# UtkuKaradeniz/scrabble-gan

Hardware: AMD Instinct MI355X
Metric: train-step images/sec @ 32×160 bs128, 1/2/4/8 GPU; % of HBM/MFMA roofline (higher is better)
Workload: dtype f32

## Files before the change

scrabble_gan_amd/csrc/conv_bf16v2.hip:

```cpp
#include "sg_conv2.h"
#include <stdlib.h>
#include <type_traits>

typedef float f32x16 __attribute__((ext_vector_type(16)));
typedef __bf16 bf16x8 __attribute__((ext_vector_type(8)));
typedef short s16x8 __attribute__((ext_vector_type(8)));
__device__ __attribute__((aligned(256))) unsigned int sg2_zero_page[64];

__device__ __forceinline__ int sg2_xcd_remap(int orig, int nwg) {
  const int q = nwg >> 3, r = nwg & 7, xcd = orig & 7;
  const int base = xcd < r ? xcd * (q + 1) : r * (q + 1) + (xcd - r) * q;
  return base + (orig >> 3);
}

__global__ __launch_bounds__(256) void k_cvt_bf16(const float* __restrict__ x, u16* __restrict__ out, long n8, int relu,
                                                  const float* __restrict__ rowscale, long rowlen) {
  for (long e = (long)blockIdx.x * blockDim.x + threadIdx.x; e < n8; e += (long)gridDim.x * blockDim.x) {
    float4 v0 = reinterpret_cast<const float4*>(x)[2 * e], v1 = reinterpret_cast<const float4*>(x)[2 * e + 1];
    if (rowscale) {
      const float s = rowscale[(8 * e) / rowlen];
      v0.x *= s; v0.y *= s; v0.z *= s; v0.w *= s; v1.x *= s; v1.y *= s; v1.z *= s; v1.w *= s;
    }
    if (relu) {
      v0.x = fmaxf(v0.x, 0.f); v0.y = fmaxf(v0.y, 0.f); v0.z = fmaxf(v0.z, 0.f); v0.w = fmaxf(v0.w, 0.f);
// ... 28 lines not shown
    const int cg = cg0 + cl;
    float s[8] = {0.f, 0.f, 0.f, 0.f, 0.f, 0.f, 0.f, 0.f};
    if (cg < c8) {
      for (long m = m0 + rl; m < m1; m += RL) {
        const float4* src = reinterpret_cast<const float4*>(x + m * C + 8 * cg);
        float4 v0 = src[0], v1 = src[1];
        if (out_plain) {
          bf16x8 hp;
          hp[0] = (__bf16)v0.x; hp[1] = (__bf16)v0.y; hp[2] = (__bf16)v0.z; hp[3] = (__bf16)v0.w;
          hp[4] = (__bf16)v1.x; hp[5] = (__bf16)v1.y; hp[6] = (__bf16)v1.z; hp[7] = (__bf16)v1.w;
          *reinterpret_cast<bf16x8*>(out_plain + m * C + 8 * cg) = hp;
        }
        if (rowscale) {
          const float f = rowscale[m / rows_per_sample];
          v0.x *= f; v0.y *= f; v0.z *= f; v0.w *= f; v1.x *= f; v1.y *= f; v1.z *= f; v1.w *= f;
        }
        bf16x8 hh;
        hh[0] = (__bf16)v0.x; hh[1] = (__bf16)v0.y; hh[2] = (__bf16)v0.z; hh[3] = (__bf16)v0.w;
        hh[4] = (__bf16)v1.x; hh[5] = (__bf16)v1.y; hh[6] = (__bf16)v1.z; hh[7] = (__bf16)v1.w;
        *reinterpret_cast<bf16x8*>(out + m * C + 8 * cg) = hh;
        s[0] += v0.x; s[1] += v0.y; s[2] += v0.z; s[3] += v0.w; s[4] += v1.x; s[5] += v1.y; s[6] += v1.z; s[7] += v1.w;
      }
    }
    if (RL > 1) {
#pragma unroll
      for (int j = 0; j < 8; ++j) red[j * 256 + threadIdx.x] = s[j];
      __syncthreads();
      for (int st = RL >> 1; st > 0; st >>= 1) {
        if (rl < st) {
#pragma unroll
          for (int j = 0; j < 8; ++j) red[j * 256 + threadIdx.x] += red[j * 256 + threadIdx.x + st * CL];
        }
        __syncthreads();
      }
#pragma unroll
      for (int j = 0; j < 8; ++j) s[j] = red[j * 256 + threadIdx.x];
      __syncthreads();
    }
    if (rl == 0 && cg < c8) {
#pragma unroll
      for (int j = 0; j < 8; ++j) atomicAdd(dbias + 8 * cg + j, s[j]);
    }
  }
}

extern "C" int sg_cvt_bf16_bias(const float* x, void* out, void* out_plain, long M, int C, const float* rowscale, long rows_per_sample,
                                float* dbias, void* stream) {
  if (!x || !out || !dbias || M < 0 || C <= 0 || (C & 7) || (rowscale && rows_per_sample <= 0)) return SG_ERR_ARG;
  if (M == 0) return SG_OK;
  long r = (M + 1023) / 1024;
  if (sg_deterministic()) r = M;
  const int rpb = (int)(r < 32 ? 32 : r);
  SG_KERNEL(k_cvt_bf16_bias, dim3((unsigned)((M + rpb - 1) / rpb)), dim3(256), 0, (hipStream_t)stream, x, (u16*)out, (u16*)out_plain, M, C,
                     rowscale, rows_per_sample, dbias, rpb);
  return sg_launch_status();
}

constexpr int SG2_BM = 256, SG2_BK = 64;
constexpr int SG2_TILE = SG2_BM * SG2_BK * 2;
constexpr int SG2_LDS = 4 * SG2_TILE;

template <int BN, int ES, bool RELU, int BMT = 256, int NWO = 0>
__global__ __launch_bounds__((NWO ? NWO : (BMT == 256 ? 8 : 4)) * 64, 2) void sg_igemm_bf16v2_kernel(const SgIgemm2Args p) {
  extern __shared__ __attribute__((aligned(1024))) unsigned char smem[];
  constexpr int BM = BMT, BK = 128 / ES;
  constexpr int NW = NWO ? NWO : (BM == 256 ? 8 : 4);
  constexpr int ATILE = BM * 128;
  constexpr int WN = BN / 64, WM = NW / WN;
  constexpr int TM = BM / WM / 32, TN = 2;
  constexpr int BQ = BN / (8 * NW);
  constexpr int AQ = BM / (8 * NW);
  static_assert(BM == 256 || (BM == 128 && (BN == 128 || (BN == 64 && ES == 4))), "tile configurations");
  static_assert(NWO == 0 || (NWO == 8 && BM == 128 && ES == 4), "eight waves: the fp32 128 x 128 tile only");
  constexpr int BTILE = BN * 128;
  const int tid = threadIdx.x;
  const int lane = tid & 63;
  const int wave = __builtin_amdgcn_readfirstlane(tid >> 6);
  const int wm = wave / WN, wn = wave % WN;

  const int M = p.Bn * p.Hg * p.Wg;
  const int HW = p.Hg * p.Wg;
  const int n_tiles = p.N / BN;
  int wg, split, nsplit;
  if ((int)blockIdx.x < p.full_tiles) {
    wg = sg2_xcd_remap(blockIdx.x, p.full_tiles);
    split = 0;
    nsplit = 1;
  } else {
    const int tail_tiles = p.n_tiles_total - p.full_tiles;
    const int u = sg2_xcd_remap(blockIdx.x - p.full_tiles, tail_tiles * p.tail_split);
    nsplit = p.tail_split;
    split = u / tail_tiles;
    wg = p.full_tiles + (u - split * tail_tiles);
  }
  const int m0 = (wg / n_tiles) * BM;
  const int n0 = (wg % n_tiles) * BN;
  const int grp = p.group_rows ? m0 / p.group_rows : 0;
  const int grp_row0 = grp * p.group_rows;
  const int kchunks = p.Ca / BK;
  const int KT_all = p.ntaps * kchunks;
  const int kt_begin = (int)(((long)KT_all * split) / nsplit);
  const int KT = (int)(((long)KT_all * (split + 1)) / nsplit) - kt_begin;

  const int lrow = lane >> 3, lslot = lane & 7;
  const unsigned char* zero = reinterpret_cast<const unsigned char*>(sg2_zero_page) + 16 * lslot;
  unsigned a_off[4], a_msk[4], b_off[4];
#pragma unroll
  for (int i = 0; i < 4; ++i) {
    const int r = (NW * i + wave) * 8 + lrow;
    const int chunk = lslot ^ ((r >> 1) & 7);
    const int m = m0 + r;
    const bool ok = m < M;
    const int mm = ok ? m - grp_row0 : 0;
    const int b = mm / HW;
    const int rem = mm - b * HW;
    const int yg = rem / p.Wg;
    const int xg = rem - yg * p.Wg;
    const int y = yg * p.a_sy, x = xg * p.a_sx;
    a_off[i] = (unsigned)ES * (unsigned)(((b * p.Ha + y) * p.Wa + x) * p.Ca) + 16u * chunk;
    unsigned mk = 0;
    for (int t = 0; t < p.ntaps; ++t) {
      const int iy = y + p.taps[t].dy, ix = x + p.taps[t].dx;
      if (ok && iy >= 0 && iy < p.Ha && ix >= 0 && ix < p.Wa) mk |= 1u << t;
    }
    a_msk[i] = mk;
    b_off[i] = (unsigned)ES * (unsigned)((n0 + (r % BN)) * p.Ca) + 16u * chunk;
  }
  int tab_a = 0, tab_w = 0;
  if (lane < p.ntaps) {
    tab_a = ES * (p.taps[lane].dy * p.Wa + p.taps[lane].dx) * p.Ca;
    tab_w = ES * p.taps[lane].w_off;
  }
  int lt = kt_begin % p.ntaps, lc0 = (kt_begin / p.ntaps) * BK;
  int lidx = 0;
  int cur_a = 0, cur_w = 0;
  unsigned cur_bit = 0;
  bool cur_live = true;
  auto set_cursor = [&]() {
    cur_live = lidx < KT;
    cur_a = __builtin_amdgcn_readlane(tab_a, lt) + ES * lc0;
    cur_w = __builtin_amdgcn_readlane(tab_w, lt) + ES * lc0;
    cur_bit = cur_live ? (1u << lt) : 0u;
  };
  set_cursor();
  auto advance = [&]() {
    ++lidx;
    ++lt;
    const bool wrap = lt >= p.ntaps;
    lt = wrap ? 0 : lt;
    lc0 += wrap ? BK : 0;
    set_cursor();
  };
  const unsigned long long a_base64 = (unsigned long long)reinterpret_cast<uintptr_t>(p.a) + (unsigned long long)grp * (unsigned long long)p.a_group_bytes;
  const unsigned long long z_base64 = (unsigned long long)reinterpret_cast<uintptr_t>(zero);
  const unsigned long long w_base64 = (unsigned long long)reinterpret_cast<uintptr_t>(p.w) + (unsigned long long)grp * (unsigned long long)p.w_group_bytes;
  auto issue_part = [&](int st, int q) {
    const bool ok = (a_msk[q] & cur_bit) != 0;
    const unsigned long long pa = a_base64 + (unsigned long long)(a_off[q] + (unsigned)cur_a);
    const unsigned lo = ok ? (unsigned)pa : (unsigned)z_base64;
    const unsigned hi = ok ? (unsigned)(pa >> 32) : (unsigned)(z_base64 >> 32);
    const unsigned char* src_a = reinterpret_cast<const unsigned char*>((uintptr_t)(((unsigned long long)hi << 32) | lo));
    const unsigned long long pb = cur_live ? w_base64 + (unsigned long long)(b_off[q] + (unsigned)cur_w) : z_base64;
    const unsigned char* src_b = reinterpret_cast<const unsigned char*>((uintptr_t)pb);
    unsigned char* dst_a = smem + st * ATILE + (NW * q + wave) * 1024;
    unsigned char* dst_b = smem + 2 * ATILE + st * BTILE + (NW * q + wave) * 1024;
    if (q < AQ)
      __builtin_amdgcn_global_load_lds((const __attribute__((address_space(1))) void*)src_a, (__attribute__((address_space(3))) void*)dst_a, 16, 0, 0);
    if (q < BQ)
      __builtin_amdgcn_global_load_lds((const __attribute__((address_space(1))) void*)src_b, (__attribute__((address_space(3))) void*)dst_b, 16, 0, 0);
  };

  f32x16 acc[TM][TN];
#pragma unroll
// ... 284 lines not shown
            idx = ((size_t)(b * p.Ho + yg * p.o_sy + p.o_oy) * p.Wo + xg * p.o_sx + p.o_ox) * p.N + n;
          }
          float v = acc[i][j][r] * oscale + bs;
          if (p.mask16) {
            if ((short)p.mask16[idx] <= 0) v = 0.f;
          } else if (p.mask && p.mask[idx] <= 0.f) {
            v = 0.f;
          }
          atomicAdd(p.out + idx, v);
        }
      }
    }
    return;
  }
#pragma unroll
  for (int i = 0; i < TM; ++i) {
    size_t idx[8];
    bool live[8];
    float4 mk32[8], prev[8];
    uint2 mk16[8];
#pragma unroll
    for (int it = 0; it < 8; ++it) {
      const int m = m0 + wm * (TM * 32) + i * 32 + 4 * it + rsub;
      live[it] = m < M;
      const int mm = live[it] ? m : 0;
      if (ident) {
        idx[it] = (size_t)mm * p.N + ncol;
      } else {
        const int b = mm / HW;
        const int rem = mm - b * HW;
        const int yg = rem / p.Wg;
        const int xg = rem - yg * p.Wg;
        idx[it] = ((size_t)(b * p.Ho + yg * p.o_sy + p.o_oy) * p.Wo + xg * p.o_sx + p.o_ox) * p.N + ncol;
      }
      if (p.mask16) mk16[it] = *reinterpret_cast<const uint2*>(p.mask16 + idx[it]);
      else if (p.mask) mk32[it] = *reinterpret_cast<const float4*>(p.mask + idx[it]);
      if (accum) prev[it] = *reinterpret_cast<const float4*>(p.out + idx[it]);
    }
#pragma unroll
    for (int j = 0; j < TN; ++j)
#pragma unroll
      for (int r = 0; r < 16; ++r) stage[((r & 3) + 8 * (r >> 2) + 4 * khalf) * 64 + j * 32 + (lane & 31)] = acc[i][j][r];
#pragma unroll
    for (int it = 0; it < 8; ++it) {
      float4 v = *reinterpret_cast<const float4*>(stage + (4 * it + rsub) * 64 + 4 * c4);
      if (!live[it]) continue;
      v.x = v.x * oscale + bsum.x; v.y = v.y * oscale + bsum.y; v.z = v.z * oscale + bsum.z; v.w = v.w * oscale + bsum.w;
      if (p.mask16) {
        if ((short)(mk16[it].x & 0xffffu) <= 0) v.x = 0.f;
        if ((short)(mk16[it].x >> 16) <= 0) v.y = 0.f;
        if ((short)(mk16[it].y & 0xffffu) <= 0) v.z = 0.f;
        if ((short)(mk16[it].y >> 16) <= 0) v.w = 0.f;
      } else if (p.mask) {
        if (mk32[it].x <= 0.f) v.x = 0.f;
        if (mk32[it].y <= 0.f) v.y = 0.f;
        if (mk32[it].z <= 0.f) v.z = 0.f;
        if (mk32[it].w <= 0.f) v.w = 0.f;
      }
      if (accum) { v.x += prev[it].x; v.y += prev[it].y; v.z += prev[it].z; v.w += prev[it].w; }
      if (relu_out) { v.x = fmaxf(v.x, 0.f); v.y = fmaxf(v.y, 0.f); v.z = fmaxf(v.z, 0.f); v.w = fmaxf(v.w, 0.f); }
      typedef __bf16 bf16x4v __attribute__((ext_vector_type(4)));
      bf16x4v h;
      if (p.out16) { h[0] = (__bf16)v.x; h[1] = (__bf16)v.y; h[2] = (__bf16)v.z; h[3] = (__bf16)v.w; }
      if (p.amax_out) {
        const float4 q = p.out ? v : make_float4((float)h[0], (float)h[1], (float)h[2], (float)h[3]);
        const float a4 = fmaxf(fmaxf(fabsf(q.x), fabsf(q.y)), fmaxf(fabsf(q.z), fabsf(q.w)));
        amx = fmaxf(amx, a4);
        if (p.amax_rowscale) amx_s = fmaxf(amx_s, a4 * fabsf(p.amax_rowscale[(m0 + wm * (TM * 32) + i * 32 + 4 * it + rsub) / HW]));
      }
      if (p.out) *reinterpret_cast<float4*>(p.out + idx[it]) = v;
      if (p.out16) *reinterpret_cast<bf16x4v*>(p.out16 + idx[it]) = h;
    }
  }
  if (p.amax_out) {
    amx = sg_wave_max(amx);
    amx_s = p.amax_rowscale ? sg_wave_max(amx_s) : amx;
    if (lane == 0) {
      sg_atomic_max_nonneg(p.amax_out, amx);
      sg_atomic_max_nonneg(p.amax_out + 1, amx_s);
    }
  }
}

__global__ __launch_bounds__(256) void k_amax_rows(const float* __restrict__ x, long rows, int N, long row0, const float* __restrict__ rowscale,
                                                   long rows_per_sample, unsigned* amax_bits) {
  const int n4 = N >> 2;
  const long total = rows * n4;
  float m0 = 0.f, m1 = 0.f;
  for (long e = (long)blockIdx.x * blockDim.x + threadIdx.x; e < total; e += (long)gridDim.x * blockDim.x) {
    const float4 v = reinterpret_cast<const float4*>(x)[e];
    const float a = fmaxf(fmaxf(fabsf(v.x), fabsf(v.y)), fmaxf(fabsf(v.z), fabsf(v.w)));
    m0 = fmaxf(m0, a);
    m1 = fmaxf(m1, rowscale ? a * fabsf(rowscale[(row0 + e / n4) / rows_per_sample]) : a);
  }
  m0 = sg_wave_max(m0);
  m1 = sg_wave_max(m1);
  if ((threadIdx.x & 63) == 0) {
    sg_atomic_max_nonneg(reinterpret_cast<float*>(amax_bits), m0);
    sg_atomic_max_nonneg(reinterpret_cast<float*>(amax_bits) + 1, m1);
  }
}

static int g2_split_override = -1;
extern "C" void sg_debug_set_splitk_v2(int n) { g2_split_override = n; }

template <int BN, int ES, bool RELU, int BMT = 256, int NWO = 0>
static int sg2_launch_bn_r(SgIgemm2Args a, hipStream_t s, long* twin_rows_done) {
  const long M = (long)a.Bn * a.Hg * a.Wg;
  const int n_tiles = a.N / BN;
  const int tiles = sg_cdiv(M, BMT) * n_tiles;
  if (tiles <= 0) return SG_OK;
  const int KT_all = a.ntaps * (a.Ca / (128 / ES));
  const bool can_split = a.out && !(a.flags & SG_RELU_OUT) && ((a.flags & SG_ACCUM) || (a.flags & SG2_IDENT_OUT));
  constexpr int CUS = BMT == 256 ? 256 : 512;
  int full = tiles, nsplit = 1;
  if (can_split && g2_split_override != 1 && KT_all >= 8) {
    const int rem = tiles % CUS;
    if (g2_split_override > 1) {
      full = 0;
      nsplit = g2_split_override < KT_all ? g2_split_override : 1;
    } else if (rem > 0) {
      const int full_c = tiles < 2 * CUS ? 0 : (tiles - rem) / n_tiles * n_tiles;
      const int tail = tiles - full_c;
      auto cost = [&](int sp) { return (double)((tail * sp + CUS - 1) / CUS) / sp * (1.0 + 0.03 * (sp - 1)); };
      int best = 1;
      double best_cost = cost(1);
      const int sp_max = KT_all / 4 < 16 ? KT_all / 4 : 16;
      for (int sp = 2; sp <= sp_max; ++sp) {
        const double c = cost(sp);
        if (c < 0.97 * best_cost) { best = sp; best_cost = c; }
      }
      if (best > 1) { full = full_c; nsplit = best; }
    }
  }
  const long row0 = nsplit > 1 ? (long)(full / n_tiles) * BMT : M;
  if (nsplit > 1 && !(a.flags & SG_ACCUM)) {
    if (hipMemsetAsync(a.out + (size_t)row0 * a.N, 0, sizeof(float) * (size_t)(M - row0) * a.N, s) != hipSuccess) return SG_ERR_LAUNCH;
  }
  a.full_tiles = full;
  a.tail_split = nsplit;
  a.n_tiles_total = tiles;
  static bool attr_done = false;
  static const int lds_pad = getenv("SG2_LDS_PAD") ? atoi(getenv("SG2_LDS_PAD")) : 0;
  const int LDS_BYTES = 2 * BMT * 128 + 2 * BN * 128 + lds_pad;
  if (!attr_done) {
    if (hipFuncSetAttribute(reinterpret_cast<const void*>(sg_igemm_bf16v2_kernel<BN, ES, RELU, BMT, NWO>), hipFuncAttributeMaxDynamicSharedMemorySize, LDS_BYTES) != hipSuccess) {
      (void)hipGetLastError();
      return SG_ERR_UNSUPPORTED;
    }
    attr_done = true;
  }
  SG_KERNEL((sg_igemm_bf16v2_kernel<BN, ES, RELU, BMT, NWO>), dim3(full + (tiles - full) * nsplit), dim3((NWO ? NWO : (BMT == 256 ? 8 : 4)) * 64), LDS_BYTES, s, a);
  if (twin_rows_done) *twin_rows_done = (a.flags & SG2_IDENT_OUT) ? row0 : (nsplit > 1 ? 0 : M);
  if (a.amax_out && nsplit > 1) {
    const bool ident = (a.flags & SG2_IDENT_OUT) != 0;
    const long r0 = ident ? row0 : 0, nrows = ident ? M - row0 : (long)a.Bn * a.Ho * a.Wo;
    const long per_sample = ident ? (long)a.Hg * a.Wg : (long)a.Ho * a.Wo;
    SG_KERNEL(k_amax_rows, dim3(sg_grid_for(nrows * (a.N / 4), 256)), dim3(256), 0, s, a.out + (size_t)r0 * a.N, nrows, a.N, r0,
                       a.amax_rowscale, per_sample, reinterpret_cast<unsigned*>(a.amax_out));
  }
  return sg_launch_status();
}

template <int BN, int ES, int BMT = 256, int NWO = 0>
static int sg2_launch_bn(const SgIgemm2Args& a, hipStream_t s, long* twin_rows_done) {
  if constexpr (ES == 1) return sg2_launch_bn_r<BN, ES, false, BMT>(a, s, twin_rows_done);
  else return (a.flags & SG_RELU_IN) ? sg2_launch_bn_r<BN, ES, true, BMT, NWO>(a, s, twin_rows_done) : sg2_launch_bn_r<BN, ES, false, BMT, NWO>(a, s, twin_rows_done);
}

static int g2_tile128 = getenv("SG2_TILE128") ? atoi(getenv("SG2_TILE128")) : 0;
extern "C" void sg_debug_set_tile128(int mode) { g2_tile128 = mode; }
static bool sg2_prefer_128(const SgIgemm2Args& a, long m_tiles) {
  return a.ntaps == 1 && a.Ca >= 1024 && m_tiles <= 1024;
}

int sg_launch_igemm_bf16v2(const SgIgemm2Args& a_in, hipStream_t s, long* twin_rows_done, int es) {
  SgIgemm2Args a = a_in;
  if ((a.Ca % (128 / es)) || (a.N % 64) || a.ntaps < 1 || a.ntaps > SG_MAX_TAPS) return SG_ERR_UNSUPPORTED;
  if (es == 1 && ((a.N % 256) || !a.amax_a || !a.amax_w)) return SG_ERR_UNSUPPORTED;
  if (a.group_rows && ((a.group_rows % 128) || a.ntaps != 1 || a.Ha != 1 || a.Wa != 1 || a.Hg != 1 || a.Wg != 1 || a.Ho != 1 || a.Wo != 1 || a.out16 ||
                       a.mask || a.mask16 || a.amax_out || (long)a.Bn % a.group_rows))
    return SG_ERR_ARG;
  const long a_bytes = (long)es * (a.group_rows ? a.group_rows : a.Bn) * a.Ha * a.Wa * a.Ca;
  long w_elems = 0;
  for (int t = 0; t < a.ntaps; ++t) w_elems = a.taps[t].w_off > w_elems ? a.taps[t].w_off : w_elems;
  w_elems += (long)a.N * a.Ca;
  if (a_bytes >= (1L << 32) - 64 || es * w_elems >= (1L << 32) - 64 || (!a.group_rows && (long)a.Bn * a.Ho * a.Wo * a.N >= (1L << 31)) ||
      (long)a.Bn * a.Hg * a.Wg >= (1L << 31) - 256)
    return SG_ERR_UNSUPPORTED;
  if (a.o_sy == 1 && a.o_sx == 1 && a.o_oy == 0 && a.o_ox == 0 && a.Ho == a.Hg && a.Wo == a.Wg) a.flags |= SG2_IDENT_OUT;
  const long m_tiles = sg_cdiv((long)a.Bn * a.Hg * a.Wg, SG2_BM);
  const bool can_split = a.out && !(a.flags & SG_RELU_OUT) && ((a.flags & SG_ACCUM) || (a.flags & SG2_IDENT_OUT)) && a.ntaps * (a.Ca / (128 / es)) >= 8;
  int bn = 0;
  double best = 1e30;
  for (int c = 256; c >= 64; c >>= 1) {
    if (a.N % c) continue;
    const long tiles = m_tiles * (a.N / c);
    const double rounds = can_split && tiles % 256 ? (tiles < 256 ? 1.0 : (double)tiles / 256.0) : (double)((tiles + 255) / 256);
    const double t_tile = es == 4 ? (c == 256 ? 1.0 : c == 128 ? 0.525 : 0.29) : es == 1 ? (c == 256 ? 1.0 : c == 128 ? 0.8 : 0.7)
                                                                                        : (c == 256 ? 1.0 : c == 128 ? 0.75 : 0.625);
    if (rounds * t_tile < 0.97 * best) { best = rounds * t_tile; bn = c; }
  }
  static const int bn_env = getenv("SG2_FORCE_BN") ? atoi(getenv("SG2_FORCE_BN")) : 0;
  if (bn_env > 0 && a.N % bn_env == 0) bn = bn_env;
  if (es == 1) {
    if (bn == 256) return sg2_launch_bn<256, 1>(a, s, twin_rows_done);
    if (bn == 128) return sg2_launch_bn<128, 1>(a, s, twin_rows_done);
    return sg2_launch_bn<64, 1>(a, s, twin_rows_done);
  }
  if (es == 4) {
    static const int w8 = getenv("SG2_W8") ? atoi(getenv("SG2_W8")) : 1;
    const long g_tiles = (long)sg_cdiv((long)a.Bn * a.Hg * a.Wg, 128) * (a.N / 128);
    if (a.group_rows && a.N % 128 == 0 && (w8 == 2 || (w8 == 1 && g_tiles < 8 * 512))) return sg2_launch_bn<128, 4, 128, 8>(a, s, twin_rows_done);
    if (a.group_rows && a.N % 128) return a.N % 64 == 0 ? sg2_launch_bn<64, 4, 128>(a, s, twin_rows_done) : SG_ERR_UNSUPPORTED;
    if (a.group_rows) return sg2_launch_bn<128, 4, 128>(a, s, twin_rows_done);
    if (bn == 256) return sg2_launch_bn<256, 4>(a, s, twin_rows_done);
    if (bn == 128) return sg2_launch_bn<128, 4>(a, s, twin_rows_done);
    return sg2_launch_bn<64, 4>(a, s, twin_rows_done);
  }
  if (a.N % 128 == 0 && bn >= 128 && (g2_tile128 == 2 || (g2_tile128 == 1 && sg2_prefer_128(a, m_tiles)))) return sg2_launch_bn<128, 2, 128>(a, s, twin_rows_done);
  if (bn == 256) return sg2_launch_bn<256, 2>(a, s, twin_rows_done);
  if (bn == 128) return sg2_launch_bn<128, 2>(a, s, twin_rows_done);
  return sg2_launch_bn<64, 2>(a, s, twin_rows_done);
}

static int finish_twin(const SgIgemm2Args& a, long rows_done, hipStream_t s) {
  if (!a.out16) return SG_OK;
  const long M = (long)a.Bn * a.Ho * a.Wo;
  if (rows_done >= M) return SG_OK;
  const long n = (M - rows_done) * a.N;
  SG_KERNEL(k_cvt_bf16, dim3(sg_grid_for(n / 8, 256)), dim3(256), 0, s, a.out + (size_t)rows_done * a.N,
                     a.out16 + (size_t)rows_done * a.N, n / 8, 0, (const float*)nullptr, 8L);
  return sg_launch_status();
}

extern "C" int sg_conv2d_fwd_bf16v2(const void* x16, const void* wp_fwd, const float* bias, const float* bias2, float* y, void* y16,
                                    int B, int H, int W, int Cin, int Cout, int kh, int kw, int pad_same, int flags, float* amax_y,
                                    void* stream) {
  if (!x16 || !wp_fwd || (!y && !y16) || (!y && (flags & SG_ACCUM)) || kh * kw > SG_MAX_TAPS) return SG_ERR_ARG;
  const int ph = pad_same ? kh / 2 : 0, pw = pad_same ? kw / 2 : 0;
  const int Ho = pad_same ? H : H - kh + 1, Wo = pad_same ? W : W - kw + 1;
  SgIgemm2Args a{};
  a.a = (const u16*)x16; a.w = (const u16*)wp_fwd; a.out = y; a.out16 = (u16*)y16; a.bias = bias; a.bias2 = bias2; a.mask = nullptr;
  a.amax_out = amax_y;
  a.Bn = B; a.Ha = H; a.Wa = W; a.Ca = Cin; a.Hg = Ho; a.Wg = Wo; a.a_sy = 1; a.a_sx = 1;
  a.Ho = Ho; a.Wo = Wo; a.N = Cout; a.o_sy = 1; a.o_sx = 1; a.o_oy = 0; a.o_ox = 0;
  a.ntaps = kh * kw; a.flags = flags;
  for (int ky = 0; ky < kh; ++ky)
    for (int kx = 0; kx < kw; ++kx) a.taps[ky * kw + kx] = SgTap{ky - ph, kx - pw, (ky * kw + kx) * Cin * Cout};
  long done = 0;
  const int rc = sg_launch_igemm_bf16v2(a, (hipStream_t)stream, &done, 2);
  return rc != SG_OK ? rc : finish_twin(a, done, (hipStream_t)stream);
}

extern "C" int sg_conv2d_bwd_data_bf16v2(const void* dy16, const void* wp_bwd, const float* mask, const void* mask16, float* dx, void* dx16,
                                         int B, int H, int W, int Cin, int Cout, int kh, int kw, int pad_same, int flags, float* amax_dx,
                                         const float* amax_rowscale, void* stream) {
  if (!dy16 || !wp_bwd || !dx || kh * kw > SG_MAX_TAPS) return SG_ERR_ARG;
  const int ph = pad_same ? kh / 2 : 0, pw = pad_same ? kw / 2 : 0;
  const int Ho = pad_same ? H : H - kh + 1, Wo = pad_same ? W : W - kw + 1;
  SgIgemm2Args a{};
  a.a = (const u16*)dy16; a.w = (const u16*)wp_bwd; a.out = dx; a.out16 = (u16*)dx16; a.mask = mask; a.mask16 = (const u16*)mask16;
  a.amax_out = amax_dx; a.amax_rowscale = amax_rowscale;
  a.Bn = B; a.Ha = Ho; a.Wa = Wo; a.Ca = Cout; a.Hg = H; a.Wg = W; a.a_sy = 1; a.a_sx = 1;
  a.Ho = H; a.Wo = W; a.N = Cin; a.o_sy = 1; a.o_sx = 1;
  a.ntaps = kh * kw; a.flags = flags;
  for (int ky = 0; ky < kh; ++ky)
    for (int kx = 0; kx < kw; ++kx) a.taps[ky * kw + kx] = SgTap{ph - ky, pw - kx, (ky * kw + kx) * Cin * Cout};
  long done = 0;
  const int rc = sg_launch_igemm_bf16v2(a, (hipStream_t)stream, &done, 2);
  return rc != SG_OK ? rc : finish_twin(a, done, (hipStream_t)stream);
}

extern "C" int sg_conv2d_fwd_v2(const float* x, const float* wt_fwd, const float* bias, const float* bias2, float* y, int B, int H,
                                int W, int Cin, int Cout, int kh, int kw, int pad_same, int flags, void* stream) {
  if (!x || !wt_fwd || !y || kh * kw > SG_MAX_TAPS) return SG_ERR_ARG;
  const int ph = pad_same ? kh / 2 : 0, pw = pad_same ? kw / 2 : 0;
  const int Ho = pad_same ? H : H - kh + 1, Wo = pad_same ? W : W - kw + 1;
  SgIgemm2Args a{};
  a.a = (const u16*)x; a.w = (const u16*)wt_fwd; a.out = y; a.bias = bias; a.bias2 = bias2;
  a.Bn = B; a.Ha = H; a.Wa = W; a.Ca = Cin; a.Hg = Ho; a.Wg = Wo; a.a_sy = 1; a.a_sx = 1;
  a.Ho = Ho; a.Wo = Wo; a.N = Cout; a.o_sy = 1; a.o_sx = 1; a.o_oy = 0; a.o_ox = 0;
  a.ntaps = kh * kw; a.flags = flags;
  for (int ky = 0; ky < kh; ++ky)
    for (int kx = 0; kx < kw; ++kx) a.taps[ky * kw + kx] = SgTap{ky - ph, kx - pw, (ky * kw + kx) * Cin * Cout};
  return sg_launch_igemm_bf16v2(a, (hipStream_t)stream, nullptr, 4);
}

extern "C" int sg_conv2d_bwd_data_v2(const float* dy, const float* w, const float* mask, float* dx, int B, int H, int W, int Cin,
                                     int Cout, int kh, int kw, int pad_same, int flags, void* stream) {
  if (!dy || !w || !dx || kh * kw > SG_MAX_TAPS) return SG_ERR_ARG;
  const int ph = pad_same ? kh / 2 : 0, pw = pad_same ? kw / 2 : 0;
  const int Ho = pad_same ? H : H - kh + 1, Wo = pad_same ? W : W - kw + 1;
  SgIgemm2Args a{};
// ... 524 lines not shown
```

scrabble_gan_amd/csrc/sg_conv2.h:

```cpp
#pragma once
#include "sg_conv.h"

typedef unsigned short u16;

#define SG2_IDENT_OUT 32

struct SgIgemm2Args {
  const u16* a;
  const u16* w;
  float* out;
  u16* out16;
  const float* bias;
  const float* bias2;
  const float* mask;
  const u16* mask16;
  const float* amax_a;
  const float* amax_w;
  float* amax_out;
  const float* amax_rowscale;
  int Bn, Ha, Wa, Ca;
  int Hg, Wg, a_sy, a_sx;
  int Ho, Wo, N, o_sy, o_sx, o_oy, o_ox;
  int ntaps, flags;
  int full_tiles, tail_split, n_tiles_total;
  int group_rows;
  long a_group_bytes, w_group_bytes;
  SgTap taps[SG_MAX_TAPS];
};

int sg_launch_igemm_bf16v2(const SgIgemm2Args& a_in, hipStream_t s, long* twin_rows_done, int es);
```

scrabble_gan_amd/ops.py:

```python
from __future__ import annotations

import os as _os
from typing import Optional, Tuple

import torch

from ._lib import call, lib

RELU_IN, ACCUM, RELU_OUT, TANH_OUT = 1, 2, 4, 8
MMA_BF16 = 256
BN_EPS = 1e-3


class KernelTimer:

    def __init__(self, only=None):
        self.records = {}
        self.shapes = {}
        self.nbytes = {}
        self.only = only
        self.roof = {}

    def wants(self, family):
        return self.only is None or any(family.startswith(p) for p in self.only)
# ... 551 lines not shown
    _chk(t, rowscale, db)
    out = torch.empty(t.shape, device=t.device, dtype=torch.bfloat16)
    plain = torch.empty(t.shape, device=t.device, dtype=torch.bfloat16) if want_plain else None
    C = t.shape[-1]
    M = t.numel() // C
    with _hbm("cvt_bf16", t, out, plain):
        call("sg_cvt_bf16_bias", _p(t), out.data_ptr(), None if plain is None else plain.data_ptr(), M, C, _p(rowscale),
             (M // rowscale.numel()) if rowscale is not None else 1, _p(db), _stream())
    return (out, plain) if want_plain else out


def grad_operand(dy: torch.Tensor, sample_scale, want_colsum: bool):
    key = (dy.untyped_storage().data_ptr(), 0 if sample_scale is None else sample_scale.data_ptr(), dy.storage_offset(), dy.numel())
    e = _TWINS.get(key)
    plain = _twin_get(dy)
    if e is None or (want_colsum and e[3] is None):
        whole = dy.storage_offset() == 0 and dy.numel() * 4 == dy.untyped_storage().nbytes()
        colsum = torch.zeros(dy.shape[-1], device=dy.device, dtype=torch.float32)
        if sample_scale is None:
            t16 = cvt_bf16_bias(dy, None, colsum)
            if plain is None:
                _twin_put(dy, t16)
        elif plain is None and whole:
            t16, p16 = cvt_bf16_bias(dy, sample_scale, colsum, want_plain=True)
            _twin_put(dy, p16)
        else:
            t16 = cvt_bf16_bias(dy, sample_scale, colsum)
        e = (dy, sample_scale, t16, colsum)
        _TWINS[key] = e
    return e[2], e[3]


def bf16_of(t: torch.Tensor) -> torch.Tensor:
    t16 = _twin_get(t)
    if t16 is None:
        t16 = cvt_bf16(t)
        _twin_put(t, t16)
    return t16


USE_F32_V2 = _os.environ.get("SG_F32_V2", "1") == "1"


F32_V2_MIN_TILES = 512


def _f32v2_ok(K: int, N: int, kh: int, kw: int, same: bool, pixels: int) -> bool:
    if not (USE_F32_V2 and CONV_DTYPE == "f32" and K % 32 == 0 and N % 64 == 0 and (same or (kh == 1 and kw == 1))):
        return False
    tiles = -(-pixels // 256) * -(-N // 256)
    return tiles >= F32_V2_MIN_TILES and (F32_V2_MIN_TILES == 0 or kh * kw * K >= 1024)


USE_WINOGRAD = _os.environ.get("SG_WINOGRAD", "1") == "1"
WINO_TILE = int(_os.environ.get("SG_WINO_TILE", "4"))
WINO_MIN_C = {2: int(_os.environ.get("SG_WINO_MIN_C", "128")), 4: int(_os.environ.get("SG_WINO4_MIN_C", "64"))}
WINO_MIN_KN = {2: int(_os.environ.get("SG_WINO_MIN_KN", "32768")), 4: int(_os.environ.get("SG_WINO4_MIN_KN", "16384"))}
WINO4_WGRAD_MIN_TILES = 128
_WINO_WS = {}
WINO_KEEP_V = _os.environ.get("SG_WINO_KEEP_V", "1") == "1"
_WINO_V = {"on": False, "map": {}}


def _wino_v_get(x: torch.Tensor, relu_in: bool, tile: int):
    e = _WINO_V["map"].get(x.untyped_storage().data_ptr())
    if e is None or e[1] != relu_in or e[2] != tile or e[0].shape[1:] != x.shape[1:]:
        return None
    per = x.shape[1] * x.shape[2] * x.shape[3]
    off = x.storage_offset() - e[0].storage_offset()
    if off < 0 or off % per or off // per + x.shape[0] > e[0].shape[0]:
        return None
    t0 = (off // per) * (x.shape[1] // tile) * (x.shape[2] // tile)
    if e[5] != _stream():
        e[3].record_stream(torch.cuda.current_stream())
    return e[3].data_ptr() + 4 * t0 * x.shape[3], e[4]


def _wino_tile(H: int, W: int) -> int:
    return 4 if (WINO_TILE == 4 and H % 4 == 0 and W % 4 == 0) else 2


WINO_ROW_GAIN = float(_os.environ.get("SG_WINO_ROW_GAIN", "0.75"))
WINO_N_MULT = int(_os.environ.get("SG_WINO_N_MULT", "64"))


def _wino_rows_ok(B, H: int, W: int, tile: int) -> bool:
    if B is None or WINO_ROW_GAIN <= 0 or DETERMINISTIC:
        return True
    T = B * (H // tile) * (W // tile)
    return (tile + 2) ** 2 * (-(-T // 128) * 128) <= WINO_ROW_GAIN * 9 * (-(-(B * H * W) // 128) * 128)


def _wino_ok(K: int, N: int, kh: int, kw: int, same: bool, H: int, W: int, B=None) -> bool:
    if not (USE_WINOGRAD and CONV_DTYPE == "f32" and kh == 3 and kw == 3 and same and H % 2 == 0 and W % 2 == 0 and K % 32 == 0 and N % WINO_N_MULT == 0):
        return False
    t = _wino_tile(H, W)
    return min(K, N) >= WINO_MIN_C[t] and K * N >= WINO_MIN_KN[t] and _wino_rows_ok(B, H, W, t)


def _wino_workspace(nbytes: int, like: torch.Tensor) -> torch.Tensor:
    key = _stream()
    buf = _WINO_WS.get(key)
    if buf is None or buf.numel() < nbytes:
        _WINO_WS.pop(key, None)
        buf = None
        buf = torch.empty(nbytes, device=like.device, dtype=torch.uint8)
        _WINO_WS[key] = buf
    return buf


def _wino_conv(a, w, out, bias, bias2, mask, K: int, N: int, relu_in: bool, flags: int, tag, ups: bool = False) -> None:
    B, H, W, _ = a.shape
    if ups:
        H, W = 2 * H, 2 * W
        flags |= UPS2_IN
    tile = _wino_tile(H, W)
    P = (tile + 2) ** 2
    fwd = tag[0] == "wino_fwd"
    u = packed_filter(w, ("wino_fwd%d" if fwd else "wino_bwd%d") % tile)
    T = B * (H // tile) * (W // tile)
    Tp = -(-T // 128) * 128
    nbytes = 4 * P * Tp * (K + N)
    s = _stream()
    keep = (fwd and _WINO_V["on"] and a.storage_offset() == 0 and _wino_wgrad_ok(K, N, 3, 3, True, H, W)
            and (tile == 2 or T >= WINO4_WGRAD_MIN_TILES))
    if keep:
        Vt = torch.empty(P * Tp * K, device=a.device, dtype=torch.float32)
        if len(_WINO_V["map"]) > 256:
            _WINO_V["map"].clear()
        _WINO_V["map"][a.untyped_storage().data_ptr()] = (a, bool(relu_in), tile, Vt, Tp, s)
        V = Vt.data_ptr()
        Mt = _wino_workspace(4 * P * Tp * N, a).data_ptr()
        if PROFILER is None:
            call("sg_wino_input", _p(a), V, B, H, W, K, int(relu_in), tile, s)
            call("sg_wino_gemm", V, _p(u), Mt, B, H, W, K, N, tile, s)
            call("sg_wino_output", Mt, _p(out), _p(bias), _p(bias2), None, B, H, W, N, flags, tile, s)
            return
    else:
        ws = _wino_workspace(nbytes, a)
        V = ws.data_ptr()
        Mt = V + 4 * P * Tp * K
    if PROFILER is None:
        if fwd:
            call("sg_conv2d_fwd_wino", _p(a), _p(u), _p(bias), _p(bias2), _p(out), B, H, W, K, N, flags | (1 if relu_in else 0), tile, V, nbytes, s)
        else:
            call("sg_conv2d_bwd_data_wino", _p(a), _p(u), _p(mask), _p(out), B, H, W, N, K, flags, tile, V, nbytes, s)
        return
    with _hbm("wino_transform", a, flops=0.0) as _:
        if PROFILER is not None and PROFILER.wants("wino_transform"):
            PROFILER.nbytes["wino_transform"] = PROFILER.nbytes.get("wino_transform", 0.0) + 4.0 * P * T * K
        if ups:
            call("sg_wino_input_ups", _p(a), V, B, H, W, K, tile, s)
        else:
            call("sg_wino_input", _p(a), V, B, H, W, K, int(relu_in), tile, s)
    with _timed("igemm_wino", 2.0 * P * Tp * K * N, False, tag):
        if PROFILER is not None and PROFILER.wants("igemm_wino"):
            PROFILER.nbytes["igemm_wino"] = PROFILER.nbytes.get("igemm_wino", 0.0) + 4.0 * P * (Tp * K + N * K + Tp * N)
        call("sg_wino_gemm", V, _p(u), Mt, B, H, W, K, N, tile, s)
    with _hbm("wino_transform", out, mask, flops=0.0):
        if PROFILER is not None and PROFILER.wants("wino_transform"):
            PROFILER.nbytes["wino_transform"] = PROFILER.nbytes.get("wino_transform", 0.0) + 4.0 * P * T * N
        call("sg_wino_output", Mt, _p(out), _p(bias), _p(bias2), _p(mask), B, H, W, N, flags & ~UPS2_IN, tile, s)


def _wino_wgrad_ok(Cin: int, Cout: int, kh: int, kw: int, same: bool, H: int, W: int) -> bool:
    if not (USE_WINOGRAD and CONV_DTYPE == "f32" and not DETERMINISTIC and kh == 3 and kw == 3 and same and H % 2 == 0 and W % 2 == 0
# ... 790 lines not shown
```

Baseline: 937.8.

## Add persistent fp32 kernel for Winograd batched GEMMs with cross-tile prefetch

Adds a persistent kernel for fp32 grouped single-tap GEMMs, the Winograd batched products. It is enabled by default and launches at most two workgroups per CU. Each workgroup loops over 128x128 output tiles and prefetches the next tile's first K chunks while storing the current tile's output. This hides per-tile prologue and epilogue latency and launch overhead, and any split-K tail is offset via block0 to the existing kernel. The cost is added complexity and possible load imbalance with the static tile stride.

```diff
diff --git a/scrabble_gan_amd/csrc/conv_bf16v2.hip b/scrabble_gan_amd/csrc/conv_bf16v2.hip
--- a/scrabble_gan_amd/csrc/conv_bf16v2.hip
+++ b/scrabble_gan_amd/csrc/conv_bf16v2.hip
@@ -134,13 +134,15 @@
   const int HW = p.Hg * p.Wg;
   const int n_tiles = p.N / BN;
   int wg, split, nsplit;
-  if ((int)blockIdx.x < p.full_tiles) {
-    wg = sg2_xcd_remap(blockIdx.x, p.full_tiles);
+  int bid = (int)blockIdx.x;
+  if constexpr (ES == 4 && BMT == 128) bid += p.block0;
+  if (bid < p.full_tiles) {
+    wg = sg2_xcd_remap(bid, p.full_tiles);
     split = 0;
     nsplit = 1;
   } else {
     const int tail_tiles = p.n_tiles_total - p.full_tiles;
-    const int u = sg2_xcd_remap(blockIdx.x - p.full_tiles, tail_tiles * p.tail_split);
+    const int u = sg2_xcd_remap(bid - p.full_tiles, tail_tiles * p.tail_split);
     nsplit = p.tail_split;
     split = u / tail_tiles;
     wg = p.full_tiles + (u - split * tail_tiles);
@@ -591,6 +593,192 @@
   }
 }
 
+template <int NW>
+__global__ __launch_bounds__(NW * 64, 2) void sg_wino_persist_kernel(const SgIgemm2Args p) {
+  extern __shared__ __attribute__((aligned(1024))) unsigned char smem[];
+  typedef unsigned long long u64;
+  constexpr int BM = 128, BN = 128, BK = 32;
+  constexpr int ATILE = BM * 128, BTILE = BN * 128;
+  constexpr int WN = BN / 64, WM = NW / WN;
+  constexpr int TM = BM / WM / 32, TN = 2;
+  constexpr int NQ = BM / (8 * NW);
+  constexpr int RP = 128 / NW;
+  static_assert(NW == 4 || NW == 8, "four or eight waves");
+  const int tid = threadIdx.x;
+  const int lane = tid & 63;
+  const int wave = __builtin_amdgcn_readfirstlane(tid >> 6);
+  const int wm = wave / WN, wn = wave % WN;
+  const int n_tiles = p.N / BN;
+  const int KT = p.Ca / BK;
+  const int KT2 = (KT + 1) & ~1;
+  const int grid = (int)gridDim.x;
+
+  auto coords = [&](int vb, int& m0, int& n0, int& grp) {
+    const int wg = sg2_xcd_remap(vb, p.full_tiles);
+    const int mt = wg / n_tiles;
+    m0 = mt * BM;
+    n0 = (wg - mt * n_tiles) * BN;
+    grp = m0 / p.group_rows;
+  };
+  auto bases = [&](int vb, u64& a64, u64& b64, bool& live) {
+    live = vb < p.full_tiles;
+    int m0, n0, grp;
+    coords(live ? vb : 0, m0, n0, grp);
+    a64 = (u64)reinterpret_cast<uintptr_t>(p.a) + (u64)grp * (u64)p.a_group_bytes + 4ull * (u64)(m0 - grp * p.group_rows) * (u64)p.Ca;
+    b64 = (u64)reinterpret_cast<uintptr_t>(p.w) + (u64)grp * (u64)p.w_group_bytes + 4ull * (u64)n0 * (u64)p.Ca;
+  };
+
+  const int lrow = lane >> 3, lslot = lane & 7;
+  const int r0 = wave * 8 + lrow;
+  const unsigned l_off = 4u * (unsigned)(r0 * p.Ca) + 16u * (unsigned)(lslot ^ ((r0 >> 1) & 7));
+  const unsigned qstride = 4u * (unsigned)(NW * 8 * p.Ca);
+  const unsigned z_off = 16u * (unsigned)lslot;
+  const u64 z_base64 = (u64)reinterpret_cast<uintptr_t>(sg2_zero_page);
+
+  int lvb = (int)blockIdx.x, lk = 0;
+  u64 a_cur, b_cur, nx_a, nx_b;
+  bool t_live, nx_live;
+  bases(lvb, a_cur, b_cur, t_live);
+  bases(lvb + grid, nx_a, nx_b, nx_live);
+  bool cur_live = t_live;
+  auto advance = [&]() {
+    ++lk;
+    const bool wrap = lk >= KT2;
+    lk = wrap ? 0 : lk;
+    lvb = wrap ? lvb + grid : lvb;
+    a_cur = wrap ? nx_a : a_cur;
+    b_cur = wrap ? nx_b : b_cur;
+    t_live = wrap ? nx_live : t_live;
+    cur_live = t_live && lk < KT;
+  };
+  auto issue_part = [&](int st, int q) {
+    const u64 kb = (u64)(unsigned)(lk * 128);
+    const u64 sa = cur_live ? a_cur + kb : z_base64;
+    const u64 sb = cur_live ? b_cur + kb : z_base64;
+    const unsigned off = cur_live ? l_off + (unsigned)q * qstride : z_off;
+    const unsigned char* src_a = reinterpret_cast<const unsigned char*>((uintptr_t)(sa + off));
+    const unsigned char* src_b = reinterpret_cast<const unsigned char*>((uintptr_t)(sb + off));
+    unsigned char* dst_a = smem + st * ATILE + (NW * q + wave) * 1024;
+    unsigned char* dst_b = smem + 2 * ATILE + st * BTILE + (NW * q + wave) * 1024;
+    __builtin_amdgcn_global_load_lds((const __attribute__((address_space(1))) void*)src_a, (__attribute__((address_space(3))) void*)dst_a, 16, 0, 0);
+    __builtin_amdgcn_global_load_lds((const __attribute__((address_space(1))) void*)src_b, (__attribute__((address_space(3))) void*)dst_b, 16, 0, 0);
+  };
+
+  f32x16 acc[TM][TN];
+  const int frow = lane & 31, khalf = lane >> 5, swz = (frow >> 1) & 7;
+  const unsigned lds0 = (unsigned)(uintptr_t)(__attribute__((address_space(3))) unsigned char*)smem;
+  typedef float v2f __attribute__((ext_vector_type(2)));
+  unsigned a4[8], b4[8];
+#pragma unroll
+  for (int s = 0; s < 8; ++s) {
+    const unsigned ko = 16u * (unsigned)(s ^ swz) + 8u * (unsigned)khalf;
+    a4[s] = lds0 + (unsigned)((wm * (TM * 32) + frow) * 128) + ko;
+    b4[s] = lds0 + (unsigned)(2 * ATILE + (wn * 64 + frow) * 128) + ko;
+  }
+  v2f af4[2][4], bf4[2][2];
+  auto mma4 = [&](int slot) {
+#pragma unroll
+    for (int e = 0; e < 2; ++e)
+#pragma unroll
+      for (int i = 0; i < TM; ++i)
+#pragma unroll
+        for (int j = 0; j < TN; ++j) acc[i][j] = __builtin_amdgcn_mfma_f32_32x32x2f32(af4[slot][i][e], bf4[slot][j][e], acc[i][j], 0, 0, 0);
+  };
+  auto mma4_dma = [&](int slot, int st) {
+#pragma unroll
+    for (int e = 0; e < 2; ++e)
+#pragma unroll
+      for (int i = 0; i < TM; ++i) {
+#pragma unroll
+        for (int j = 0; j < TN; ++j) acc[i][j] = __builtin_amdgcn_mfma_f32_32x32x2f32(af4[slot][i][e], bf4[slot][j][e], acc[i][j], 0, 0, 0);
+        if (e == 0) {
+          __builtin_amdgcn_sched_barrier(0);
+#pragma unroll
+          for (int q = i * NQ / TM; q < (i + 1) * NQ / TM; ++q) issue_part(st, q);
+          __builtin_amdgcn_sched_barrier(0);
+        }
+      }
+    advance();
+  };
+#define SG4_K_TILE_LAST(st, sn)                                                              \
+  do {                                                                                       \
+    SG4_STEP(st, 1, 1, 0);                                                                   \
+    SG4_STEP(st, 2, 0, 1);                                                                   \
+    SG4_STEP(st, 3, 1, 0);                                                                   \
+    SG4_STEP(st, 4, 0, 1);                                                                   \
+    SG4_STEP(st, 5, 1, 0);                                                                   \
+    SG4_STEP(st, 6, 0, 1);                                                                   \
+    SG4_STEP(st, 7, 1, 0);                                                                   \
+    asm volatile("s_waitcnt vmcnt(0) lgkmcnt(0)" ::: "memory");                              \
+    __builtin_amdgcn_s_barrier();                                                            \
+    SG4_READ_FRAGS(sn, 0, 0);                                                                \
+    __builtin_amdgcn_sched_barrier(0);                                                       \
+    mma4(1);                                                                                 \
+    __builtin_amdgcn_sched_barrier(0);                                                       \
+    asm volatile("s_waitcnt lgkmcnt(0)" ::: "memory");                                       \
+    __builtin_amdgcn_sched_barrier(0);                                                       \
+  } while (0)
+
+  const int sbyte = wave * (RP * 256);
+  float* stage = reinterpret_cast<float*>(smem + (sbyte < ATILE ? ATILE + sbyte : 2 * ATILE + BTILE + (sbyte - ATILE)));
+  const int c4 = lane & 15, rsub = lane >> 4;
+
+  {
+#pragma unroll
+    for (int q = 0; q < NQ; ++q) issue_part(0, q);
+    advance();
+    asm volatile("s_waitcnt vmcnt(0)" ::: "memory");
+    __builtin_amdgcn_s_barrier();
+#pragma unroll
+    for (int q = 0; q < NQ; ++q) issue_part(1, q);
+    advance();
+    SG4_READ_FRAGS(0, 0, 0);
+  }
+  for (int cvb = (int)blockIdx.x;; cvb += grid) {
+    bases(lvb + grid, nx_a, nx_b, nx_live);
+#pragma unroll
+    for (int i = 0; i < TM; ++i)
+#pragma unroll
+      for (int j = 0; j < TN; ++j)
+#pragma unroll
+        for (int r = 0; r < 16; ++r) acc[i][j][r] = 0.f;
+    for (int kt = 2; kt < KT2; kt += 2) {
+      SG4_K_TILE(0, 1);
+      SG4_K_TILE(1, 0);
+    }
+    SG4_K_TILE(0, 1);
+    SG4_K_TILE_LAST(1, 0);
+
+    int m0, n0, grp;
+    coords(cvb, m0, n0, grp);
+    float* out_t = p.out + ((size_t)m0 * p.N + n0);
+#pragma unroll
+    for (int ps = 0; ps < 2; ++ps) {
+      constexpr int NR = NW == 4 ? 16 : 8;
+      const int i = NW == 4 ? ps : 0, rb = NW == 4 ? 0 : 8 * ps;
+#pragma unroll
+      for (int j = 0; j < TN; ++j)
+#pragma unroll
+        for (int rr = 0; rr < NR; ++rr) stage[((rr & 3) + 8 * (rr >> 2) + 4 * khalf) * 64 + j * 32 + (lane & 31)] = acc[i][j][rb + rr];
+#pragma unroll
+      for (int it = 0; it < RP / 4; ++it) {
+        float4 v = *reinterpret_cast<const float4*>(stage + (4 * it + rsub) * 64 + 4 * c4);
+        v.x += 0.f; v.y += 0.f; v.z += 0.f; v.w += 0.f;
+        const int row = wm * (TM * 32) + ps * RP + 4 * it + rsub;
+        *reinterpret_cast<float4*>(out_t + ((size_t)row * p.N + wn * 64 + 4 * c4)) = v;
+      }
+    }
+    if (cvb + grid >= p.full_tiles) break;
+    asm volatile("s_waitcnt lgkmcnt(0)" ::: "memory");
+    __builtin_amdgcn_s_barrier();
+    __builtin_amdgcn_sched_barrier(0);
+#pragma unroll
+    for (int q = 0; q < NQ; ++q) issue_part(1, q);
+    advance();
+    __builtin_amdgcn_sched_barrier(0);
+  }
+}
+
 __global__ __launch_bounds__(256) void k_amax_rows(const float* __restrict__ x, long rows, int N, long row0, const float* __restrict__ rowscale,
                                                    long rows_per_sample, unsigned* amax_bits) {
   const int n4 = N >> 2;
@@ -612,6 +800,20 @@
 
 static int g2_split_override = -1;
 extern "C" void sg_debug_set_splitk_v2(int n) { g2_split_override = n; }
+
+static int g2_wino_persist = getenv("SG_WINO_PERSIST") ? atoi(getenv("SG_WINO_PERSIST")) : 1;
+static int g2_wino_persist_wgs = getenv("SG_WINO_PERSIST_WGS") ? atoi(getenv("SG_WINO_PERSIST_WGS")) : 0;
+extern "C" void sg_debug_set_wino_persist(int mode, int wgs) {
+  g2_wino_persist = mode;
+  g2_wino_persist_wgs = wgs;
+}
+static bool sg2_wino_persist_wanted(const SgIgemm2Args& a, long M) {
+  if (g2_wino_persist <= 0) return false;
+  if (!a.group_rows || a.ntaps != 1 || a.flags != SG2_IDENT_OUT || !a.out || a.out16 || a.bias || a.bias2 || a.mask || a.mask16 || a.amax_out ||
+      (M % 128) || (a.N % 128) || (a.Ca % 32))
+    return false;
+  return true;
+}
 
 template <int BN, int ES, bool RELU, int BMT = 256, int NWO = 0>
 static int sg2_launch_bn_r(SgIgemm2Args a, hipStream_t s, long* twin_rows_done) {
@@ -649,6 +851,32 @@
   a.full_tiles = full;
   a.tail_split = nsplit;
   a.n_tiles_total = tiles;
+  a.block0 = 0;
+  if constexpr (ES == 4 && BMT == 128 && BN == 128 && !RELU) {
+    if (full > 0 && sg2_wino_persist_wanted(a, M)) {
+      constexpr int PNW = NWO ? NWO : 4;
+      static bool pattr_done = false;
+      static int slots = 0;
+      if (!pattr_done) {
+        int dev = 0, cus = 0;
+        if (hipGetDevice(&dev) != hipSuccess || hipDeviceGetAttribute(&cus, hipDeviceAttributeMultiprocessorCount, dev) != hipSuccess || cus <= 0) cus = 256;
+        if (hipFuncSetAttribute(reinterpret_cast<const void*>(sg_wino_persist_kernel<PNW>), hipFuncAttributeMaxDynamicSharedMemorySize, 4 * 128 * 128) != hipSuccess) {
+          (void)hipGetLastError();
+          return SG_ERR_UNSUPPORTED;
+        }
+        slots = 2 * cus;
+        pattr_done = true;
+      }
+      int grid = full < slots ? full : slots;
+      if (g2_wino_persist_wgs > 0 && grid > g2_wino_persist_wgs) grid = g2_wino_persist_wgs;
+      SG_KERNEL((sg_wino_persist_kernel<PNW>), dim3(grid), dim3(PNW * 64), 4 * 128 * 128, s, a);
+      if (full == tiles) {
+        if (twin_rows_done) *twin_rows_done = M;
+        return sg_launch_status();
+      }
+      a.block0 = full;
+    }
+  }
   static bool attr_done = false;
   static const int lds_pad = getenv("SG2_LDS_PAD") ? atoi(getenv("SG2_LDS_PAD")) : 0;
   const int LDS_BYTES = 2 * BMT * 128 + 2 * BN * 128 + lds_pad;
@@ -659,7 +887,7 @@
     }
     attr_done = true;
   }
-  SG_KERNEL((sg_igemm_bf16v2_kernel<BN, ES, RELU, BMT, NWO>), dim3(full + (tiles - full) * nsplit), dim3((NWO ? NWO : (BMT == 256 ? 8 : 4)) * 64), LDS_BYTES, s, a);
+  SG_KERNEL((sg_igemm_bf16v2_kernel<BN, ES, RELU, BMT, NWO>), dim3(full - a.block0 + (tiles - full) * nsplit), dim3((NWO ? NWO : (BMT == 256 ? 8 : 4)) * 64), LDS_BYTES, s, a);
   if (twin_rows_done) *twin_rows_done = (a.flags & SG2_IDENT_OUT) ? row0 : (nsplit > 1 ? 0 : M);
   if (a.amax_out && nsplit > 1) {
     const bool ident = (a.flags & SG2_IDENT_OUT) != 0;
@@ -677,6 +905,8 @@
   else return (a.flags & SG_RELU_IN) ? sg2_launch_bn_r<BN, ES, true, BMT, NWO>(a, s, twin_rows_done) : sg2_launch_bn_r<BN, ES, false, BMT, NWO>(a, s, twin_rows_done);
 }
 
+static int g2_w8 = getenv("SG2_W8") ? atoi(getenv("SG2_W8")) : 1;
+extern "C" void sg_debug_set_w8(int mode) { g2_w8 = mode; }
 static int g2_tile128 = getenv("SG2_TILE128") ? atoi(getenv("SG2_TILE128")) : 0;
 extern "C" void sg_debug_set_tile128(int mode) { g2_tile128 = mode; }
 static bool sg2_prefer_128(const SgIgemm2Args& a, long m_tiles) {
@@ -718,7 +948,7 @@
     return sg2_launch_bn<64, 1>(a, s, twin_rows_done);
   }
   if (es == 4) {
-    static const int w8 = getenv("SG2_W8") ? atoi(getenv("SG2_W8")) : 1;
+    const int w8 = g2_w8;
     const long g_tiles = (long)sg_cdiv((long)a.Bn * a.Hg * a.Wg, 128) * (a.N / 128);
     if (a.group_rows && a.N % 128 == 0 && (w8 == 2 || (w8 == 1 && g_tiles < 8 * 512))) return sg2_launch_bn<128, 4, 128, 8>(a, s, twin_rows_done);
     if (a.group_rows && a.N % 128) return a.N % 64 == 0 ? sg2_launch_bn<64, 4, 128>(a, s, twin_rows_done) : SG_ERR_UNSUPPORTED;
diff --git a/scrabble_gan_amd/csrc/sg_conv2.h b/scrabble_gan_amd/csrc/sg_conv2.h
--- a/scrabble_gan_amd/csrc/sg_conv2.h
+++ b/scrabble_gan_amd/csrc/sg_conv2.h
@@ -26,6 +26,7 @@
   int group_rows;
   long a_group_bytes, w_group_bytes;
   SgTap taps[SG_MAX_TAPS];
+  int block0;
 };
 
 int sg_launch_igemm_bf16v2(const SgIgemm2Args& a_in, hipStream_t s, long* twin_rows_done, int es);
diff --git a/scrabble_gan_amd/ops.py b/scrabble_gan_amd/ops.py
--- a/scrabble_gan_amd/ops.py
+++ b/scrabble_gan_amd/ops.py
@@ -657,6 +657,10 @@
 
 WINO_ROW_GAIN = float(_os.environ.get("SG_WINO_ROW_GAIN", "0.75"))
 WINO_N_MULT = int(_os.environ.get("SG_WINO_N_MULT", "64"))
+
+
+def set_wino_persist(mode: int, wgs: int = 0) -> None:
+    lib().sg_debug_set_wino_persist(int(mode), int(wgs))
 
 
 def _wino_rows_ok(B, H: int, W: int, tile: int) -> bool:
```

Result: faster. 961.4 (median of 6 runs) (+2.5%).
